# manyeyes/K2TransducerAsr

Hardware: AMD Instinct MI355X
Metric: RTFx (audio-sec/wall-sec) offline Zipformer greedy (higher is better)
Workload: dtype f32

## Files before the change

### k2transducerasr_amd/csrc/engine.cpp

```cpp
#include <cstring>
#include <thread>

#include "engine.h"
#include "lattice_ref.h"
#include "ctc_lattice_ref.h"
#include "ctc_prefix_bias_ref.h"
#include "ctc_prefix_ref.h"
#include "hotwords.h"
#include "ngram_lm.h"

#include <climits>
#include <cmath>

namespace k2hip {

namespace {
constexpr int kTailFrames = 19;
}

Engine::Engine(const std::string& weights, const char* overrides, int device) : device_(device) {
    tunables_init_from_env();
    model_.reset(new Model(weights, overrides));
    int n = 0;
    if (hipGetDeviceCount(&n) != hipSuccess || n <= 0)
// ... 208 lines not shown
        K2_HIP(hipMemcpyAsync(d_y, y.data(), sizeof(long long) * y.size(), hipMemcpyHostToDevice, stream_));
        Ctx t;
        t.stream = stream_;
        decoder_rows_wide(t, w, d_y, N, d_out);
        K2_HIP(hipMemcpyAsync(got.data(), d_out, sizeof(float) * got.size(), hipMemcpyDeviceToHost, stream_));
        K2_HIP(hipStreamSynchronize(stream_));
        for (int n = 0; n < N; n++) {
            const long long row = (y[2 * n] + 1) * V + y[2 * n + 1];
            K2_HIP(copy_blocking(want.data(), w.dec_table + row * w.J, sizeof(float) * w.J, hipMemcpyDeviceToHost));
            for (int k = 0; k < w.J; k++) *mismatched += memcmp(&want[k], &got[(size_t)n * w.J + k], sizeof(float)) != 0;
        }
    } catch (...) {
        (void)hipFree(d_y);
        (void)hipFree(d_out);
        throw;
    }
    (void)hipFree(d_y);
    (void)hipFree(d_out);
}

float* Engine::encoder_embed(const Ctx& c, const float* x, int B, int T, int* T50) {
    const Model& m = *model_;
    const int F0 = 80, T1 = T - 2, T2 = (T1 - 3) / 2 + 1, F2 = (F0 - 3) / 2 + 1, T3 = T2 - 2, F3 = (F2 - 3) / 2 + 1;
    K2_REQUIRE(T3 > 0, "encoder: %d input frames are too few (need >= 9)", T);
    Arena& ar = *c.arena;
    const int D0 = m.cfg().dim[0];
    float* out = ar.take<float>((int64_t)B * T3 * D0);
    int64_t mark = ar.mark();
    float* a1 = ar.take<float>((int64_t)B * T1 * F0 * 8);
    conv0_swoosh(c, x, m.w("encoder_embed.conv.0.weight"), m.w("encoder_embed.conv.0.bias"), a1, B, T, F0);
    c.add_flops(0, 2.0 * B * T1 * (double)F0 * 8 * 9, 0);
    float* a2 = ar.take<float>((int64_t)B * T2 * F2 * 32);
    {
        GemmArgs g;
        g.A = a1; g.W = m.w("encoder_embed.conv.4.weight#ohwi"); g.ldw = 72; g.bias = m.w("encoder_embed.conv.4.bias");
        g.C = a2; g.ldc = 32; g.M = B * T2 * F2; g.N = 32; g.K = 72; g.act = ACT_SWOOSH_R;
        g.cv_Fout = F2; g.cv_Tout = T2; g.cv_Tin = T1; g.cv_Fin = F0; g.cv_C = 8; g.cv_st = 2; g.cv_sf = 2;
        g.seg_len = 24; g.seg_stride = F0 * 8;
        gemm(c, g);
    }
    float* a3 = ar.take<float>((int64_t)B * T3 * F3 * 128);
    {
        GemmArgs g;
        g.A = a2; g.W = m.w("encoder_embed.conv.7.weight#ohwi"); g.ldw = 288; g.bias = m.w("encoder_embed.conv.7.bias");
        g.C = a3; g.ldc = 128; g.M = B * T3 * F3; g.N = 128; g.K = 288; g.act = ACT_SWOOSH_R;
        g.cv_Fout = F3; g.cv_Tout = T3; g.cv_Tin = T2; g.cv_Fin = F2; g.cv_C = 32; g.cv_st = 1; g.cv_sf = 2;
        g.seg_len = 96; g.seg_stride = F2 * 32;
        gemm(c, g);
    }
    const int npix = B * T3 * F3;
    float* dw = ar.take<float>((int64_t)npix * 128);
    dwconv7x7(c, a3, m.w("encoder_embed.convnext.depthwise_conv.weight#kc"), m.w("encoder_embed.convnext.depthwise_conv.bias"),
              dw, B, T3, T3, 3, F3, 128);
    float* hid = ar.take<float>((int64_t)npix * 384);
    linear(c, dw, 128, m.w("encoder_embed.convnext.pointwise_conv1.weight"), m.w("encoder_embed.convnext.pointwise_conv1.bias"),
           hid, 384, npix, 128, 384, ACT_SWOOSH_L);
    linear(c, hid, 384, m.w("encoder_embed.convnext.pointwise_conv2.weight"), m.w("encoder_embed.convnext.pointwise_conv2.bias"),
           a3, 128, npix, 384, 128, ACT_NONE, a3, 128);
    float* lin = ar.take<float>((int64_t)B * T3 * D0);
    linear(c, a3, F3 * 128, m.w("encoder_embed.out.weight#fc"), m.w("encoder_embed.out.bias"), lin, D0, B * T3, F3 * 128, D0);
    biasnorm(c, lin, m.w("encoder_embed.out_norm.bias"), m.w("encoder_embed.out_norm.log_scale"), out, B * T3, D0);
    ar.rewind(mark);
    *T50 = T3;
    return out;
}

const float* Engine::pos_proj_cached(const Ctx& c, int layer, const float* pe, int pe_dim, const float* W, int rows, int ncols) {
    if (c.dry) return nullptr;
    std::lock_guard<std::mutex> lk(cache_mu_);
    const auto key = std::make_pair(layer, rows);
    auto it = pp_cache_.find(key);
    if (it != pp_cache_.end()) return it->second;
    const size_t bytes = sizeof(float) * (size_t)rows * ncols;
    if (pp_cache_bytes_ + bytes > ((size_t)1 << 30)) {
        synchronize();
        for (auto& kv : pp_cache_) (void)hipFree(kv.second);
        pp_cache_.clear();
        pp_cache_bytes_ = 0;
    }
    float* pp = nullptr;
    K2_HIP(hipMalloc(&pp, bytes));
    Ctx plain = c;
    plain.instrument = false;
    plain.gemm_log = nullptr;
    linear(plain, pe, pe_dim, W, nullptr, pp, ncols, rows, pe_dim, ncols);
    K2_HIP(hipStreamSynchronize(c.stream));
    pp_cache_[key] = pp;
    pp_cache_bytes_ += bytes;
    return pp;
}

void Engine::encoder_layer(const Ctx& c, int si, int li, int gl, float* x, const float* pe, int B, int T, const StreamSite* site,
                           const LayerTail* tail) {
    const Model& m = *model_;
    const Config& cf = m.cfg();
    const int D = cf.dim[si], F = cf.ff[si], H = cf.heads[si], vh = cf.vhd[si], K = cf.kern[si], qh = cf.qhd[si], ph = cf.phd[si];
    const int L = site ? cf.left[si] : 0, M = B * T, KL = L + T, KLp = (KL + 3) & ~3, inproj = (2 * qh + ph) * H, Hc = 3 * D / 4, HV = H * vh;
    char p[96];
    snprintf(p, sizeof p, "encoder.encoders.%d.layers.%d.", si, li);
    auto w = [&](const char* suffix) { return m.w(std::string(p) + suffix); };
    auto wk = [&](const char* fmt, int k) {
        char name[96];
        snprintf(name, sizeof name, fmt, k);
        return w(name);
    };
    Arena& ar = *c.arena;
    int64_t mark = ar.mark();
    const long long SS = lay_.floats_per_stream;
    auto ring = [&](long long off) {
        RingRef r;
        r.pool = online_pool_; r.slot_stride = SS; r.off = off; r.slots = site->d_slots; r.chunks = site->d_chunks;
// ... 1583 lines not shown
            if (kcat) attn_stream(c, qkp, ld, kcat, pp, plen, aw, B, Tc, Lc, KLp, H, ds, left50);
            else attn_stream_ring(c, qkp, ld, r, pp, plen, aw, B, Tc, Lc, KLp, H, ds, left50);
        } else if (name == "glu_causal_conv") {
            float *x2 = P(), *pool = P();
            const long long ss = L(), off = L();
            const int* slots = reinterpret_cast<const int*>(P());
            float *wc = P(), *bc = P(), *ww = P(), *bw = P(), *sc = P(), *y = P();
            const int B = I(), Tc = I(), D = I(), K = I();
            glu_causal_conv(c, x2, pool, ss, off, slots, wc, bc, ww, bw, sc, y, B, Tc, D, K);
        } else if (name == "gemm") {
            GemmArgs g;
            g.M = I(); g.N = I(); g.K = I();
            g.lda = I(); g.ldw = I(); g.ldc = I(); g.ldr = I();
            g.act = I(); g.act_cols = I(); g.w_kn = I();
            g.nb0 = I(); g.nb1 = I();
            g.sA0 = L(); g.sA1 = L(); g.sW0 = L(); g.sW1 = L(); g.sC0 = L(); g.sC1 = L(); g.sR0 = L(); g.sR1 = L();
            g.sBias0 = L();
            g.cv_Fout = I(); g.cv_Tout = I(); g.cv_Tin = I(); g.cv_Fin = I(); g.cv_C = I(); g.cv_st = I(); g.cv_sf = I();
            g.seg_len = I(); g.seg_stride = I();
            g.res_div = I(); g.act_after_res = I();
            g.glu = I(); g.glu_cols = I();
            g.ldm = I(); g.sM0 = L(); g.sM1 = L();
            g.ld_orig = I();
            const int cfg = I(), res_is_C = I();
            const long long oA = L(), oW = L(), oR = L(), oC = L(), oM = L(), oO = L();
            float *A = P(), *W = P(), *bias = P(), *res = P(), *C = P();
            const int* skip = reinterpret_cast<const int*>(P());
            float *mul = P(), *orig = P(), *scale = P();
            int* plan_out = reinterpret_cast<int*>(P());
            K2_REQUIRE(A && W && C && plan_out && buf_bytes[n_bufs - 1] >= 20, "debug_op_run gemm: A, W, C and a plan buffer of 5 ints are needed");
            K2_REQUIRE(!(res_is_C && res), "debug_op_run gemm: res_is_C takes no res buffer");
            K2_REQUIRE(oA >= 0 && oW >= 0 && oR >= 0 && oC >= 0 && oM >= 0 && oO >= 0, "debug_op_run gemm: negative offset");
            if (res_is_C) res = C;
            g.A = A + oA; g.W = W + oW; g.bias = bias; g.res = res ? res + oR : nullptr; g.C = C + oC;
            g.skip_if_zero = skip;
            g.mul = mul ? mul + oM : nullptr;
            g.byp_orig = orig ? orig + oO : nullptr; g.byp_scale = scale;
            GemmForceGuard force(cfg);
            const GemmPlan pl = plan_gemm(g, gemm_force());
            const int rep[5] = {(int)pl.family, pl.idx, pl.BM, pl.BN, pl.mode};
            K2_HIP(copy_blocking(plan_out, rep, sizeof rep, hipMemcpyHostToDevice));
            gemm(c, g);
        } else if (name == "gemm_glu_causal_conv") {
            float *x = P(), *wg = P(), *bg = P(), *pool = P();
            const long long ss = L(), off = L();
            const int* slots = reinterpret_cast<const int*>(P());
            float *wc = P(), *bc = P(), *ww = P(), *bw = P(), *sc = P(), *y = P();
            const int B = I(), Tc = I(), D = I(), K = I();
            int* entry_out = reinterpret_cast<int*>(P());
            K2_REQUIRE(entry_out && buf_bytes[n_bufs - 1] >= 4, "debug_op_run gemm_glu_causal_conv: an entry buffer of 1 int is needed");
            const int entry = glu_conv_ring_entry(B, Tc, D, K);
            K2_HIP(copy_blocking(entry_out, &entry, sizeof entry, hipMemcpyHostToDevice));
            took = gemm_glu_causal_conv(c, x, wg, bg, pool, ss, off, slots, wc, bc, ww, bw, sc, y, B, Tc, D, K);
        } else if (name == "biasnorm") {
            float *x = P(), *bias = P(), *ls = P(), *y = P();
            const int M = I(), D = I();
            biasnorm(c, x, bias, ls, y, M, D);
        } else if (name == "bypass") {
            float *orig = P(), *x = P(), *scale = P(), *y = P();
            const int M = I(), D = I();
            bypass(c, orig, x, scale, y, M, D);
        } else if (name == "biasnorm_bypass") {
            float *x = P(), *orig = P(), *nb = P(), *ls = P(), *scale = P(), *y = P();
            const int M = I(), D = I();
            biasnorm_bypass(c, x, orig, nb, ls, scale, y, M, D);
        } else if (name == "biasnorm_bypass_downsample") {
            float *x = P(), *orig = P(), *nb = P(), *ls = P(), *scale = P(), *y = P(), *bias2 = P(), *xd2 = P();
            const int B = I(), T = I(), D = I(), ds2 = I(), D2 = I();
            biasnorm_bypass_downsample(c, x, orig, nb, ls, scale, y, bias2, xd2, B, T, D, ds2, D2);
        } else if (name == "downsample") {
            float *x = P(), *bias = P(), *y = P();
            const int B = I(), T = I(), D = I(), ds = I(), Din = I();
            downsample(c, x, bias, y, B, T, D, ds, Din);
        } else if (name == "downsample_full") {
            FullDimSegs s;
            s.n = I();
            K2_REQUIRE(s.n >= 1 && s.n <= 8, "debug_op_run downsample_full: %d segments", s.n);
            for (int k = 0; k < s.n; k++) s.ld[k] = I();
            for (int k = 0; k < s.n; k++) s.col1[k] = I();
            s.lz_Td = I(); s.lz_ds = I(); s.lz_Do = I();
            for (int k = 0; k < s.n; k++) s.src[k] = P();
            s.lz_orig = P(); s.lz_xd = P(); s.lz_scale = P();
            float *bias = P(), *y = P();
            const int B = I(), T = I(), D = I(), ds = I();
            downsample_full(c, s, bias, y, B, T, D, ds);
        } else if (name == "upsample_combine") {
            float *orig = P(), *xd = P(), *scale = P(), *y = P();
            const int B = I(), T = I(), Td = I(), D = I(), ds = I(), Dorig = I();
            upsample_combine(c, orig, xd, scale, y, B, T, Td, D, ds, Dorig);
        } else if (name == "upsample_combine_downsample") {
            float *orig = P(), *xd = P(), *scale = P(), *y = P(), *bias2 = P(), *xd2 = P();
            const int B = I(), T = I(), Td = I(), D = I(), ds = I(), Dorig = I(), D2 = I(), ds2 = I();
            upsample_combine_downsample(c, orig, xd, scale, y, bias2, xd2, B, T, Td, D, ds, Dorig, D2, ds2);
        } else if (name == "glu_dwconv1d_swoosh" || name == "glu_dwconv1d_dswish" || name == "dwconv1d_swoosh") {
            float *x = P(), *w = P(), *b = P(), *y = P();
            const int B = I(), T = I(), D = I(), K = I();
            if (name == "glu_dwconv1d_swoosh") glu_dwconv1d_swoosh(c, x, w, b, y, B, T, D, K);
            else if (name == "glu_dwconv1d_dswish") glu_dwconv1d_dswish(c, x, w, b, y, B, T, D, K);
            else dwconv1d_swoosh(c, x, w, b, y, B, T, D, K);
        } else if (name == "dwconv7x7") {
            float *x = P(), *w = P(), *b = P(), *y = P();
            const int B = I(), Tin = I(), Tout = I(), tpad = I(), F = I(), C = I();
            dwconv7x7(c, x, w, b, y, B, Tin, Tout, tpad, F, C);
        } else if (name == "conformer_qprep") {
            float *qkv = P(), *bu = P(), *bv = P(), *qu = P(), *qv = P();
            const int M = I(), D = I();
// ... 545 lines not shown
```

### k2transducerasr_amd/csrc/gemm.hip

```cpp
#include <algorithm>
#include <cmath>
#include <cstdlib>
#include <map>
#include <mutex>
#include <type_traits>

#include "act.h"
#include "kernels.h"

#pragma clang diagnostic ignored "-Winline-asm"

namespace k2hip {

typedef float f32x16 __attribute__((ext_vector_type(16)));
typedef float f32x4 __attribute__((ext_vector_type(4)));

namespace {


__device__ __forceinline__ float apply_act(float v, int act) {
    switch (act) {
        case ACT_SWOOSH_L: return swoosh_l(v);
        case ACT_SWOOSH_R: return swoosh_r(v);
        case ACT_TANH: {
// ... 1316 lines not shown
#undef K2_STAMP
}

template <int NT, int NW = 4>
__global__ __launch_bounds__(64 * NW) void gemm_f32_mfma_skinny(GemmArgs g) {
    if (g.skip_if_zero && *g.skip_if_zero == 0) return;
    __shared__ __attribute__((aligned(16))) float red[NW][NT][64][4];
    const int tid = threadIdx.x, lane = tid & 63, wave = tid >> 6;
    const int r = lane & 15, q = lane >> 4;
    const int m0 = blockIdx.x * 16, n0 = blockIdx.y * (16 * NT);
    const int Kw = g.K / NW, kbeg = wave * Kw;
    const float* __restrict__ ap = g.A + (long long)min(m0 + r, g.M - 1) * g.lda + kbeg + 4 * q;
    const float* __restrict__ wp[NT];
#pragma unroll
    for (int j = 0; j < NT; j++) wp[j] = g.W + (long long)min(n0 + 16 * j + r, g.N - 1) * g.ldw + kbeg + 4 * q;
    f32x4 acc[NT];
#pragma unroll
    for (int j = 0; j < NT; j++) acc[j] = f32x4{0.f, 0.f, 0.f, 0.f};
    constexpr int UN = NT <= 3 ? 4 : 2;
    for (int k = 0; k < Kw; k += 16 * UN) {
        float4 a4[UN], w4[UN][NT];
#pragma unroll
        for (int u = 0; u < UN; u++) {
            const int kk = min(k + 16 * u, Kw - 16);
            const float m = (k + 16 * u < Kw) ? 1.f : 0.f;
            a4[u] = *reinterpret_cast<const float4*>(ap + kk);
            a4[u].x *= m; a4[u].y *= m; a4[u].z *= m; a4[u].w *= m;
#pragma unroll
            for (int j = 0; j < NT; j++) w4[u][j] = *reinterpret_cast<const float4*>(wp[j] + kk);
        }
#pragma unroll
        for (int u = 0; u < UN; u++)
#pragma unroll
            for (int e = 0; e < 4; e++)
#pragma unroll
                for (int j = 0; j < NT; j++) {
                    const float av = e == 0 ? a4[u].x : e == 1 ? a4[u].y : e == 2 ? a4[u].z : a4[u].w;
                    const float bv = e == 0 ? w4[u][j].x : e == 1 ? w4[u][j].y : e == 2 ? w4[u][j].z : w4[u][j].w;
                    acc[j] = __builtin_amdgcn_mfma_f32_16x16x4f32(av, bv, acc[j], 0, 0, 0);
                }
    }
#pragma unroll
    for (int j = 0; j < NT; j++) *reinterpret_cast<f32x4*>(&red[wave][j][lane][0]) = acc[j];
    __syncthreads();
    for (int j = wave; j < NT; j += NW) {
        float vals[4];
#pragma unroll
        for (int e = 0; e < 4; e++) {
            float v = red[0][j][lane][e] + red[1][j][lane][e] + red[2][j][lane][e] + red[3][j][lane][e];
            if (NW == 8) v += (red[4][j][lane][e] + red[5][j][lane][e]) + (red[6][j][lane][e] + red[7][j][lane][e]);
            vals[e] = v;
        }
        epilogue_rows<4, Rows16>(g, vals, m0 + 4 * q, n0 + 16 * j + r, g.C, g.res, vals, false, nullptr, g.bias);
    }
}

template <int BM, int BN, int WM, int WN, int NST = 3>
void launch_dma(const Ctx& ctx, const GemmArgs& a) {
    dim3 grid(cdiv(a.N, BN), cdiv(a.M, BM), a.nb0 * a.nb1);
    size_t lds = sizeof(float) * NST * (BM + BN) * 32;
    static LdsAttrOnce lds_attr;
    lds_attr.ensure(gemm_f32_mfma_dma<BM, BN, WM, WN, NST>, (int)lds);
    hipLaunchKernelGGL((gemm_f32_mfma_dma<BM, BN, WM, WN, NST>), grid, dim3(64 * (BM / WM) * (BN / WN)), lds, ctx.stream, a);
}

template <int BM, int BN, int KS, int NST, int LW, int PF = 0>
void launch_ring(const Ctx& ctx, const GemmArgs& a) {
    dim3 grid(cdiv(a.N, BN), cdiv(a.M, BM), a.nb0 * a.nb1);
    size_t lds = sizeof(float) * std::max((size_t)NST * KS * (BM + BN) * 32, KS > 1 ? (size_t)KS * (BM / 32) * (BN / 32) * 1024 : (size_t)0) + (PF ? 256 : 0);
    static LdsAttrOnce lds_attr;
    lds_attr.ensure(gemm_f32_mfma_ring<BM, BN, KS, NST, LW, PF>, (int)lds);
    hipLaunchKernelGGL((gemm_f32_mfma_ring<BM, BN, KS, NST, LW, PF>), grid, dim3(64 * ((BM / 32) * (BN / 32) * KS + LW + PF)), lds, ctx.stream, a);
}

template <int BM, int BN, int KS, int NST, int PF = 0>
void launch_ring_conv(const Ctx& ctx, const GemmArgs& a) {
    dim3 grid(cdiv(a.N, BN), cdiv(a.M, BM), 1);
    const int pad = a.cf_K >> 1, Kc = (a.cf_K + 1) >> 1, CH = BN / 2;
    const size_t conv_fl = (size_t)(BM / a.cf_Tc) * CH * (pad + a.cf_Tc) + (size_t)CH * (Kc | 1) + (size_t)CH * a.cf_K;
    size_t lds = sizeof(float) * std::max({(size_t)NST * KS * (BM + BN) * 32, KS > 1 ? (size_t)KS * (BM / 32) * (BN / 32) * 1024 : (size_t)0, conv_fl}) + (PF ? 256 : 0);
    static LdsAttrOnce lds_attr;
    lds_attr.ensure(gemm_f32_mfma_ring<BM, BN, KS, NST, 0, PF, true>, (int)lds);
    hipLaunchKernelGGL((gemm_f32_mfma_ring<BM, BN, KS, NST, 0, PF, true>), grid, dim3(64 * ((BM / 32) * (BN / 32) * KS + PF)), lds, ctx.stream, a);
}

template <int BM, int BN, int WM, int WN, int NST>
void launch_pipe(const Ctx& ctx, const GemmArgs& a) {
    dim3 grid(cdiv(a.N, BN), cdiv(a.M, BM), 1);
    size_t lds = sizeof(float) * NST * (BM + BN) * 32;
    static LdsAttrOnce lds_attr;
    lds_attr.ensure(gemm_f32_mfma_pipe<BM, BN, WM, WN, NST>, (int)lds);
    K2_REQUIRE((long long)a.M * a.lda < (1ll << 29) && (long long)a.N * a.ldw < (1ll << 29), "pipe: operand too large for 31-bit lane byte offsets");
    K2_REQUIRE(a.K % 32 == 0 && a.K >= 32 * (NST - 1), "pipe: K %d too short for %d stages", a.K, NST);
    hipLaunchKernelGGL((gemm_f32_mfma_pipe<BM, BN, WM, WN, NST>), grid, dim3(64 * (BM / WM) * (BN / WN)), lds, ctx.stream, a);
}

template <int BM, int BN, int WM, int WN, int NST>
void launch_p16(const Ctx& ctx, const GemmArgs& a) {
    dim3 grid(cdiv(a.N, BN), cdiv(a.M, BM), 1);
    size_t lds = sizeof(float) * NST * (BM + BN) * 32;
    static LdsAttrOnce lds_attr;
    lds_attr.ensure(gemm_f32_mfma_p16<BM, BN, WM, WN, NST>, (int)lds);
    K2_REQUIRE((long long)a.M * a.lda < (1ll << 29) && (long long)a.N * a.ldw < (1ll << 29), "p16: operand too large for 31-bit lane byte offsets");
    K2_REQUIRE(a.K % 32 == 0 && a.K >= 32 * (NST - 1) && !a.glu, "p16: K %d too short for %d stages, or a gated epilogue", a.K, NST);
    hipLaunchKernelGGL((gemm_f32_mfma_p16<BM, BN, WM, WN, NST>), grid, dim3(64 * (BM / WM) * (BN / WN)), lds, ctx.stream, a);
}
// ... 81 lines not shown
            }
            break;
        case GemmFamily::SKINNY3:
            hipLaunchKernelGGL(gemm_f32_mfma_skinny<3>, dim3(cdiv(a.M, 16), 1), dim3(256), 0, ctx.stream, b);
            break;
        case GemmFamily::SKINNY6:
            hipLaunchKernelGGL(gemm_f32_mfma_skinny<6>, dim3(cdiv(a.M, 16), cdiv(a.N, 96)), dim3(256), 0, ctx.stream, b);
            break;
        case GemmFamily::SKINNY6_8:
            hipLaunchKernelGGL((gemm_f32_mfma_skinny<6, 8>), dim3(cdiv(a.M, 16), cdiv(a.N, 96)), dim3(512), 0, ctx.stream, b);
            break;
    }
    K2_HIP(hipGetLastError());
    if (ctx.instrument && ctx.gemm_log)
        ctx.gemm_log->push_back({a.M, a.N, a.K, a.nb0 * a.nb1, a.act, a.res != nullptr, gemm_kind(a, p), 0.f});
    if (ctx.instrument) K2_HIP(hipEventRecord(ctx.next_event(), ctx.stream));
}

bool gemm_glu_causal_conv(const Ctx& ctx, const float* x, const float* wg, const float* bg, float* pool, long long slot_stride, long long off,
                          const int* slots, const float* wc, const float* bc, const float* ww, const float* bw, const float* sc, float* y, int B,
                          int Tc, int D, int K) {
    const int M = B * Tc, N = 2 * D;
    const int entry = glu_conv_ring_entry(B, Tc, D, K);
    if (entry < 0) return false;
    const double fl = 2.0 * M * (double)N * D;
    ctx.add_flops(fl, 2.0 * M * (double)D * (K + (K + 1) / 2), 1);
    if (ctx.dry) return true;
    GemmArgs g;
    g.A = x; g.lda = D; g.W = wg; g.ldw = D; g.bias = bg; g.C = y; g.ldc = D; g.M = M; g.N = N; g.K = D;
    g.cf_pool = pool; g.cf_stride = slot_stride; g.cf_off = off; g.cf_slots = slots;
    g.cf_wc = wc; g.cf_bc = bc; g.cf_ww = ww; g.cf_bw = bw; g.cf_sc = sc; g.cf_Tc = Tc; g.cf_K = K;
    g.xcd_panels = tunables().xcd_panels;
    if (ctx.instrument) K2_HIP(hipEventRecord(ctx.next_event(), ctx.stream));
    if (ctx.instrument && ctx.gemm_log) ctx.gemm_log->push_back({M, N, D, 1, 0, 0, 64, 0.f});
    switch (entry) {
        case 16: launch_ring_conv_entry<16>(ctx, g); break;
        case 17: launch_ring_conv_entry<17>(ctx, g); break;
        case 12: launch_ring_conv_entry<12>(ctx, g); break;
        default: launch_ring_conv_entry<8>(ctx, g); break;
    }
    K2_HIP(hipGetLastError());
    if (ctx.instrument) K2_HIP(hipEventRecord(ctx.next_event(), ctx.stream));
    return true;
}

void linear(const Ctx& ctx, const float* A, int lda, const float* W, const float* bias, float* C, int ldc, int M, int K,
            int N, int act, const float* res, int ldr) {
    GemmArgs g;
    g.A = A; g.lda = lda; g.W = W; g.ldw = K; g.bias = bias; g.C = C; g.ldc = ldc;
    g.M = M; g.N = N; g.K = K; g.act = act; g.res = res; g.ldr = ldr;
    gemm(ctx, g);
}

}
```

### k2transducerasr_amd/csrc/kernels.h

```cpp
#pragma once
#include "ctc_prefix_layout.h"
#include "common.h"

namespace k2hip {

#ifdef K2HIP_DEV
#define K2HIP_DEV_SWITCH(name, def) int name = def
#else
#define K2HIP_DEV_SWITCH(name, def) static constexpr int name = def
#endif
struct Tunables {
    int no_glu_epilogue = 0;
    int attn_long = 0;
    int no_fused_av = 0;
    int fused_vproj_min_t = 4;
    int no_fused_vproj = 0;
    int no_fused_conv = 0;
    int conformer_gemm_scores = 0;
    int dw7_tiled = 0;
    int dw1d_tt = 0;
    int lstm_seq = 0;
    int greedy_one_part = 0;
    int greedy_parts = 0;
    int beam_launches = 0;
    int beam_parts = 0;
    int beam_hyp_global = 0;
    int beam_trace = 0;
    int search_rounds = -1;
    int test_greedy_timeout = 0;
    int decoder_table_mb = 1024;
    int screen_min_v = 1024;
    int screen_count = 0;
    int max_streams = 0;
    K2HIP_DEV_SWITCH(gemm_cfg, -1);
    K2HIP_DEV_SWITCH(xcd_panels, 0);
    K2HIP_DEV_SWITCH(greedy_stamps, 0);
    K2HIP_DEV_SWITCH(conformer_stamps, 0);
};
void tunables_init_from_env();
const Tunables& tunables();
bool tunables_set(const char* env_name, int value);

struct GemmStats {
    double flops = 0;
    double total_flops = 0;
    int launches = 0;
    float ms = 0;
};

struct GemmLaunchRec {
    int M, N, K, batch, act, res, kind;
    float us;
};

struct GreedyLaunch;
struct Ctx {
    std::vector<GemmLaunchRec>* gemm_log = nullptr;
    GreedyLaunch* greedy_rec = nullptr;
    hipStream_t stream = nullptr;
    Arena* arena = nullptr;
    bool dry = false;
    bool one_part = false;
    bool instrument = false;
    GemmStats* stats = nullptr;
    std::vector<hipEvent_t>* evpool = nullptr;
    int* evused = nullptr;
    hipEvent_t next_event() const {
        if ((size_t)*evused == evpool->size()) {
            hipEvent_t e;
            K2_HIP(hipEventCreate(&e));
// ... 56 lines not shown
#define K2_PIPE_TABLE(X)                                                                                                       \
    X(0, 128, 64, 64, 32, 3) X(1, 128, 64, 32, 32, 3) X(2, 128, 128, 64, 64, 3) X(3, 128, 128, 64, 32, 3) X(4, 128, 64, 64, 32, 4)  \
    X(5, 64, 64, 32, 32, 3) X(6, 128, 128, 64, 64, 4) X(7, 64, 128, 32, 64, 3) X(8, 128, 128, 32, 32, 3) X(9, 128, 64, 32, 32, 4) \
    X(10, 64, 64, 64, 32, 3) X(11, 64, 64, 32, 64, 3) X(12, 256, 64, 64, 32, 3) X(13, 128, 32, 32, 32, 3) X(14, 128, 32, 64, 32, 3)
#define K2_P16_TABLE(X) X(0, 64, 96, 32, 48, 3) X(1, 128, 96, 64, 48, 3) X(2, 64, 192, 32, 96, 3) X(3, 32, 96, 16, 48, 3)
#define K2_RING_TABLE(X)                                                                                        \
    X(0, 128, 64, 1, 2, 0, 0) X(1, 128, 64, 1, 3, 0, 0) X(2, 128, 64, 1, 2, 0, 1) X(3, 128, 64, 1, 3, 0, 1) X(4, 128, 64, 1, 4, 0, 1)   \
    X(5, 64, 64, 1, 3, 0, 0) X(6, 64, 64, 1, 3, 0, 1) X(7, 64, 64, 1, 4, 0, 1) X(8, 64, 64, 2, 3, 0, 0) X(9, 64, 64, 2, 3, 0, 1)      \
    X(10, 64, 64, 4, 2, 0, 0) X(11, 64, 64, 4, 2, 0, 1) X(12, 32, 64, 2, 3, 0, 0) X(13, 32, 64, 4, 3, 0, 0) X(14, 32, 64, 4, 3, 0, 1)  \
    X(15, 32, 32, 4, 3, 0, 0) X(16, 32, 32, 4, 4, 0, 1) X(17, 64, 32, 4, 3, 0, 0) X(18, 128, 128, 1, 2, 0, 0) X(19, 128, 128, 1, 2, 0, 1) \
    X(20, 64, 128, 1, 3, 0, 0) X(21, 64, 128, 1, 3, 0, 1) X(22, 64, 96, 1, 3, 0, 0) X(23, 64, 96, 1, 3, 0, 1) X(24, 128, 96, 1, 2, 0, 1) \
    X(25, 128, 64, 1, 3, 2, 0) X(26, 128, 64, 1, 3, 2, 1) X(27, 128, 64, 2, 2, 0, 1) X(28, 64, 96, 2, 3, 0, 0) X(29, 64, 96, 2, 2, 0, 0) \
    X(30, 64, 96, 2, 2, 0, 1) X(31, 128, 96, 1, 3, 0, 0) X(32, 128, 96, 1, 3, 0, 1)
struct RingCfg { int BM, BN, KS, NST, LW, PF; };
#define X(i, bm, bn, ks, nst, lw, pf) {bm, bn, ks, nst, lw, pf},
constexpr RingCfg kRing[] = {K2_RING_TABLE(X)};
#undef X
#define K2_DMA_TABLE(X)                                                                                                          \
    X(0, 128, 128, 64, 32, 3) X(5, 128, 64, 32, 32, 2) X(8, 128, 64, 32, 32, 4) X(9, 64, 64, 32, 32, 2) X(10, 64, 64, 32, 32, 3) \
    X(11, 64, 96, 32, 32, 2) X(20, 32, 32, 32, 32, 4) X(21, 32, 64, 32, 32, 4)
#define K2_REG_TABLE(X)                                                                                                           \
    X(0, 128, 128, 64, 32, 32) X(1, 128, 128, 64, 32, 64) X(2, 64, 64, 32, 32, 32) X(3, 64, 64, 32, 32, 64) X(4, 128, 64, 32, 32, 64) \
    X(5, 128, 64, 32, 32, 32) X(12, 128, 32, 32, 32, 32)
enum GemmMode { MODE_PLAIN = 0, MODE_CONV = 1, MODE_WKN = 2 };

enum class GemmFamily { REG, DMA, PIPE, P16, RING, SKINNY3, SKINNY6, SKINNY6_8 };
struct GemmPlan {
    GemmFamily family = GemmFamily::REG;
    int idx = 0;
    int mode = MODE_PLAIN;
    int ablate = 0;
    int BM = 0, BN = 0, waves = 0;
};
struct GemmForce {
    enum Kind { AUTO, CFG, RING, PIPE, P16 } kind = AUTO;
    int idx = -1;
    int ablate = 0;
    bool dma = true;
};
GemmForce decode_gemm_force(int code);
GemmPlan plan_gemm(const GemmArgs& a, const GemmForce& f);
int gemm_kind(const GemmArgs& a, const GemmPlan& p);
int glu_conv_ring_entry(int B, int Tc, int D, int K);
void debug_force_gemm_cfg(int code);
GemmForce gemm_force();
struct GemmForceGuard {
    explicit GemmForceGuard(int code) { debug_force_gemm_cfg(code); }
    ~GemmForceGuard() { debug_force_gemm_cfg(-1); }
    GemmForceGuard(const GemmForceGuard&) = delete;
    GemmForceGuard& operator=(const GemmForceGuard&) = delete;
};
void linear(const Ctx& ctx, const float* A, int lda, const float* W, const float* bias, float* C, int ldc, int M, int K,
            int N, int act = ACT_NONE, const float* res = nullptr, int ldr = 0);

struct RingRef {
    float* pool = nullptr;
    long long slot_stride = 0;
    long long off = 0;
    const int* slots = nullptr;
    const int* chunks = nullptr;
};

void attn_scores_softmax(const Ctx& ctx, const float* qkp, int ld, const float* pp, float* aw, int B, int T, int Tp, int H, int qh = 32,
                         int koff0 = -1, int poff0 = -1);

bool attn_av_out(const Ctx& ctx, const float* aw, const float* v, const float* wout, const float* bias, float* x, int B, int T, int KL, int Tp,
                 int H, int vh, int D);
bool attn_av_out_ring(const Ctx& ctx, const float* aw, const RingRef& vals, const float* newrows, const float* wout, const float* bias, float* x,
                      int B, int T, int KL, int Tp, int H, int vh, int D);
void attn_proj_av_out_ring(const Ctx& ctx, const float* aw, const RingRef& vals, const float* xin, const float* win, const float* bin,
                           const float* wout, const float* bias, float* xout, int B, int T, int KL, int Tp, int H, int vh, int D);

void nonlin_av_out_ring(const Ctx& ctx, const float* aw, const RingRef& cache, const float* hid, int ldh, const float* wout, const float* bias,
                        float* x, int B, int T, int KL, int Tp, int Hc, int D);

void pad_logfloor(const Ctx& ctx, const float* packed, const long long* d_off, const long long* d_len, float* out, int B,
                  long long L);
void pad_logfloor_dense(const Ctx& ctx, const float* feats, long long n_each, float* out, int B, long long L);
void conv0_swoosh(const Ctx& ctx, const float* x, const float* w, const float* b, float* y, int B, int T, int F);
void act_forms(const Ctx& ctx, const float* x, float* y_lean, float* y_libm, int act, long long n);
void conv0_pad1_dswish(const Ctx& ctx, const float* x, const float* w, const float* b, float* y, int B, int T, int F);
void dwconv7x7(const Ctx& ctx, const float* x, const float* w_kc, const float* b, float* y, int B, int Tin, int Tout, int tpad,
               int F, int C);
void biasnorm(const Ctx& ctx, const float* x, const float* bias, const float* log_scale, float* y, int M, int D);
void biasnorm_bypass(const Ctx& ctx, const float* x, const float* orig, const float* nbias, const float* log_scale,
                     const float* scale, float* y, int M, int D);
void biasnorm_bypass_downsample(const Ctx& ctx, const float* x, const float* orig, const float* nbias, const float* log_scale, const float* scale,
                                float* y, const float* bias2, float* xd2, int B, int T, int D, int ds2, int D2);
struct LayerTail {
    const float* bias2 = nullptr;
    float* xd2 = nullptr;
    int ds2 = 1, D2 = 0;
};
void bypass(const Ctx& ctx, const float* orig, const float* x, const float* scale, float* y, int M, int D);
void glu_sigmoid(const Ctx& ctx, const float* x, float* y, int M, int D);
void tanh_gate(const Ctx& ctx, const float* x, float* y, int M, int Hc);
void dwconv1d_swoosh(const Ctx& ctx, const float* x, const float* w_kd, const float* b, float* y, int B, int T, int D, int K);
void glu_dwconv1d_swoosh(const Ctx& ctx, const float* x2, const float* w_kd, const float* b, float* y, int B, int T, int D,
                          int K);
void glu_dwconv1d_dswish(const Ctx& ctx, const float* x2, const float* w_kd, const float* b, float* y, int B, int T, int D,
                          int K);
void conv0_nopad_dswish(const Ctx& ctx, const float* x, const float* w, const float* b, float* y, int B, int T, int F);
void lstm_cell(const Ctx& ctx, const float* gx, long long ldgx, const float* gh, int ldgh, float* c, float* hf, int B, int Hh);
void add_inplace(const Ctx& ctx, float* a, const float* b, long long n);
void lstm_cell_rows(const Ctx& ctx, const float* gates, float* c, float* hf, int rows, int Hh);
void lstm_add_frame(const Ctx& ctx, const float* Y, long long SY, const float* hp, long long pstride, int S, float* h, float* x1, int n, int B,
// ... 343 lines not shown
```

### k2transducerasr_amd/csrc/online_engine.cpp

```cpp
#include <climits>
#include <cmath>

#include "engine.h"
#include "ctc_prefix_ref.h"

namespace k2hip {

void Engine::online_ensure_pool() {
    if (online_pool_) return;
    const Config& c = model_->cfg();
    K2_REQUIRE(c.streaming || c.lstm, "this model is not a streaming export (metadata 'streaming' != 1)");
    OnlineLayout& L = lay_;
    long long off = 0;
    if (c.conformer) {
        L.nl = c.nlayer[0];
        L.floats_per_stream = ((long long)c.nlayer[0] * (c.left[0] + c.kern[0] - 1) * c.dim[0] + 63) / 64 * 64;
        online_cap_ = 256;
        if (tunables().max_streams > 0) online_cap_ = tunables().max_streams;
        K2_HIP(hipSetDevice(device_));
        K2_HIP(hipMalloc(&online_pool_, sizeof(float) * (size_t)L.floats_per_stream * online_cap_));
        for (int i = online_cap_ - 1; i >= 0; i--) free_slots_.push_back(i);
        return;
    }
    if (c.lstm) {
// ... 161 lines not shown
    const float cl = sqrtf((float)pd), ls = (float)pd / (2.0f * (float)M_PI), logcl = logf(cl);
    for (int n = 0; n < n2; n++) {
        float x = (float)(n - (Tc + L - 1));
        float sg = (float)((x > 0.f) - (x < 0.f));
        float xa = atanf(cl * sg * (logf(fabsf(x) + cl) - logcl) / ls);
        for (int k = 0; k < pd / 2; k++) {
            pe[(size_t)n * pd + 2 * k] = cosf(xa * (float)(k + 1));
            pe[(size_t)n * pd + 2 * k + 1] = sinf(xa * (float)(k + 1));
        }
        pe[(size_t)n * pd + pd - 1] = 1.0f;
    }
    float* d = nullptr;
    K2_HIP(hipMalloc(&d, pe.size() * sizeof(float)));
    K2_HIP(copy_blocking(d, pe.data(), pe.size() * sizeof(float), hipMemcpyHostToDevice));
    pe_cache_[key] = d;
    return d;
}

float* Engine::encoder_embed_stream(const Ctx& c, const float* x, const int* d_slots, int B, int T, int* Tc_out) {
    const Model& m = *model_;
    const int F0 = 80, T1 = T - 2, T2 = (T1 - 3) / 2 + 1, F2 = (F0 - 3) / 2 + 1, T3 = T2 - 2, F3 = (F2 - 3) / 2 + 1, Tc = T3 - 3;
    K2_REQUIRE(Tc > 0 && F3 == 19, "streaming embed: chunk of %d frames unsupported", T);
    Arena& ar = *c.arena;
    const int D0 = m.cfg().dim[0];
    float* out = ar.take<float>((int64_t)B * Tc * D0);
    int64_t mark = ar.mark();
    float* a1 = ar.take<float>((int64_t)B * T1 * F0 * 8);
    conv0_swoosh(c, x, m.w("encoder_embed.conv.0.weight"), m.w("encoder_embed.conv.0.bias"), a1, B, T, F0);
    float* a2 = ar.take<float>((int64_t)B * T2 * F2 * 32);
    {
        GemmArgs g;
        g.A = a1; g.W = m.w("encoder_embed.conv.4.weight#ohwi"); g.ldw = 72; g.bias = m.w("encoder_embed.conv.4.bias");
        g.C = a2; g.ldc = 32; g.M = B * T2 * F2; g.N = 32; g.K = 72; g.act = ACT_SWOOSH_R;
        g.cv_Fout = F2; g.cv_Tout = T2; g.cv_Tin = T1; g.cv_Fin = F0; g.cv_C = 8; g.cv_st = 2; g.cv_sf = 2;
        g.seg_len = 24; g.seg_stride = F0 * 8;
        gemm(c, g);
    }
    float* a3 = ar.take<float>((int64_t)B * T3 * F3 * 128);
    {
        GemmArgs g;
        g.A = a2; g.W = m.w("encoder_embed.conv.7.weight#ohwi"); g.ldw = 288; g.bias = m.w("encoder_embed.conv.7.bias");
        g.C = a3; g.ldc = 128; g.M = B * T3 * F3; g.N = 128; g.K = 288; g.act = ACT_SWOOSH_R;
        g.cv_Fout = F3; g.cv_Tout = T3; g.cv_Tin = T2; g.cv_Fin = F2; g.cv_C = 32; g.cv_st = 1; g.cv_sf = 2;
        g.seg_len = 96; g.seg_stride = F2 * 32;
        gemm(c, g);
    }
    float* cat = ar.take<float>((int64_t)B * (T3 + 3) * F3 * 128);
    const int npix = B * Tc * F3;
    float* byp = ar.take<float>((int64_t)npix * 128);
    convnext_cat(c, a3, online_pool_, lay_.floats_per_stream, lay_.embed, d_slots, cat, byp, B, T3, Tc, F3, 128);
    float* dw = ar.take<float>((int64_t)npix * 128);
    dwconv7x7(c, cat, m.w("encoder_embed.convnext.depthwise_conv.weight#kc"), m.w("encoder_embed.convnext.depthwise_conv.bias"), dw, B,
              T3 + 3, Tc, 0, F3, 128);
    float* hid = ar.take<float>((int64_t)npix * 384);
    linear(c, dw, 128, m.w("encoder_embed.convnext.pointwise_conv1.weight"), m.w("encoder_embed.convnext.pointwise_conv1.bias"), hid, 384,
           npix, 128, 384, ACT_SWOOSH_L);
    linear(c, hid, 384, m.w("encoder_embed.convnext.pointwise_conv2.weight"), m.w("encoder_embed.convnext.pointwise_conv2.bias"), byp, 128,
           npix, 384, 128, ACT_NONE, byp, 128);
    float* lin = ar.take<float>((int64_t)B * Tc * D0);
    linear(c, byp, F3 * 128, m.w("encoder_embed.out.weight#fc"), m.w("encoder_embed.out.bias"), lin, D0, B * Tc, F3 * 128, D0);
    biasnorm(c, lin, m.w("encoder_embed.out_norm.bias"), m.w("encoder_embed.out_norm.log_scale"), out, B * Tc, D0);
    ar.rewind(mark);
    *Tc_out = Tc;
    return out;
}

float* Engine::online_encoder_zip2(const Ctx& c, const float* d_x, const int* d_slots, const long long* d_plen, const int* d_chunks, int B) {
    const int Tp = online_frames_per_chunk();
    int Tc = 0;
    float* x = encoder_embed_stream(c, d_x, d_slots, B, model_->cfg().chunk_T, &Tc);
    K2_REQUIRE((Tc + 1) / 2 == Tp, "internal: chunk yields %d frames, expected %d", (Tc + 1) / 2, Tp);
    const StreamSite site{d_slots, d_plen, d_chunks};
    FullDimSegs segs;
    encoder_stacks(c, x, B, Tc, &site, -1, nullptr, nullptr, &segs);
    return encoder_head(c, segs, B, Tc, nullptr);
}

void Engine::online_step(const int* slots, const float* const* chunks, const long long* hyps, const long long* plens, const int* nchunks, int B,
                         int64_t* tokens, int32_t* ts, int32_t* n_tokens, const int* fifo_heads) {
    online_step_impl(slots, chunks, hyps, plens, nchunks, B, tokens, ts, n_tokens, fifo_heads, nullptr);
}
void Engine::online_step_beam(const int* slots, const float* const* chunks, const long long* plens, const int* nchunks, int B, int K,
                              const int* beam_in, int* beam_out, const int* fifo_heads) {
    K2_REQUIRE(K >= 1 && K <= kMaxBeam, "online beam search: beam %d out of range [1,%d]", K, kMaxBeam);
    K2_REQUIRE(!model_->cfg().ctc, "online beam search: a CTC model runs its own search");
    std::vector<long long> hyps(2 * (size_t)B, K2HIP_BLANK_ID);
    OnlineBeamIO io{K, beam_in, beam_out, nullptr};
    online_step_impl(slots, chunks, hyps.data(), plens, nchunks, B, nullptr, nullptr, nullptr, fifo_heads, &io);
}
void Engine::online_step_beam_hw(const int* slots, const float* const* chunks, const long long* plens, const int* nchunks, int B, int K,
                                 const int* beam_in, int* beam_out, const BeamHwIO& hw, const int* fifo_heads) {
    K2_REQUIRE(K >= 1 && K <= kMaxBeam, "online beam search: beam %d out of range [1,%d]", K, kMaxBeam);
    K2_REQUIRE(!model_->cfg().ctc, "online beam search: a CTC model runs its own search");
    std::vector<long long> hyps(2 * (size_t)B, K2HIP_BLANK_ID);
    OnlineBeamIO io{K, beam_in, beam_out, &hw};
    online_step_impl(slots, chunks, hyps.data(), plens, nchunks, B, nullptr, nullptr, nullptr, fifo_heads, &io);
}
void Engine::online_step_ctc_prefix(const int* slots, const float* const* chunks, const long long* plens, const int* nchunks, int B, int K,
                                    const int* cp_in, int* cp_out, const int* fifo_heads) {
    K2_REQUIRE(K >= 1 && K <= kMaxBeam, "online ctc prefix search: beam %d out of range [1,%d]", K, kMaxBeam);
    K2_REQUIRE(model_->cfg().ctc, "online ctc prefix search: the model has no CTC head");
    const CtcPrefixResumeLayout L{K, online_frames_per_chunk()};
    ctc_prefix_chunk_check_args(B, L.Tc, model_->cfg().V, nullptr, K, cp_in, L.in_ints(), L.in_e(), L.in_rel());
    std::vector<long long> hyps(2 * (size_t)B, K2HIP_BLANK_ID);
    OnlineCtcPrefixIO io{K, cp_in, cp_out};
    online_step_impl(slots, chunks, hyps.data(), plens, nchunks, B, nullptr, nullptr, nullptr, fifo_heads, nullptr, &io);
}
void Engine::online_step_impl(const int* slots, const float* const* chunks, const long long* hyps, const long long* plens, const int* nchunks,
                              int B, int64_t* tokens, int32_t* ts, int32_t* n_tokens, const int* fifo_heads, const OnlineBeamIO* beam,
                              const OnlineCtcPrefixIO* cpx) {
    online_ensure_pool();
// ... 146 lines not shown
```

### k2transducerasr_amd/csrc/tunables.cpp

```cpp
#include <cstdlib>
#include <cstring>
#include <mutex>

#include "kernels.h"

namespace k2hip {

namespace {
constexpr int kMaxDev = 64;
std::mutex g_util_mu[kMaxDev];
hipStream_t g_util_stream[kMaxDev] = {};
hipError_t util_device(int* dev) {
    hipError_t e = hipGetDevice(dev);
    if (e != hipSuccess) return e;
    return (*dev < 0 || *dev >= kMaxDev) ? hipErrorInvalidDevice : hipSuccess;
}
hipError_t util_stream(int dev, hipStream_t* s) {
    if (!g_util_stream[dev]) {
        hipError_t e = hipStreamCreateWithFlags(&g_util_stream[dev], hipStreamNonBlocking);
        if (e != hipSuccess) return e;
    }
    *s = g_util_stream[dev];
    return hipSuccess;
}
}
hipError_t copy_blocking(void* dst, const void* src, size_t bytes, hipMemcpyKind kind) {
    if (bytes == 0) return hipSuccess;
    int dev = 0;
    hipError_t e = util_device(&dev);
    if (e != hipSuccess) return e;
    std::lock_guard<std::mutex> lk(g_util_mu[dev]);
    hipStream_t s = nullptr;
    e = util_stream(dev, &s);
    if (e != hipSuccess) return e;
    e = hipMemcpyAsync(dst, src, bytes, kind, s);
    if (e != hipSuccess) return e;
    return hipStreamSynchronize(s);
}
hipError_t fill_blocking(void* dst, int value, size_t bytes) {
    if (bytes == 0) return hipSuccess;
    int dev = 0;
    hipError_t e = util_device(&dev);
    if (e != hipSuccess) return e;
    std::lock_guard<std::mutex> lk(g_util_mu[dev]);
    hipStream_t s = nullptr;
    e = util_stream(dev, &s);
    if (e != hipSuccess) return e;
    e = hipMemsetAsync(dst, value, bytes, s);
    if (e != hipSuccess) return e;
    return hipStreamSynchronize(s);
}

namespace {
Tunables g_t;
bool g_init = false;
struct Entry {
    const char* env;
    int Tunables::*field;
    bool flag;
};
const Entry kEntries[] = {
    {"K2HIP_NO_GLU_EPILOGUE", &Tunables::no_glu_epilogue, true},
    {"K2HIP_ATTN_LONG", &Tunables::attn_long, true},
    {"K2HIP_NO_FUSED_AV", &Tunables::no_fused_av, true},
    {"K2HIP_NO_FUSED_VPROJ", &Tunables::no_fused_vproj, true},
    {"K2HIP_FUSED_VPROJ_MIN_T", &Tunables::fused_vproj_min_t, false},
    {"K2HIP_NO_FUSED_CONV", &Tunables::no_fused_conv, true},
    {"K2HIP_CONFORMER_GEMM_SCORES", &Tunables::conformer_gemm_scores, true},
    {"K2HIP_DW7_TILED", &Tunables::dw7_tiled, true},
    {"K2HIP_DW1D_TT", &Tunables::dw1d_tt, false},
    {"K2HIP_LSTM_SEQ", &Tunables::lstm_seq, true},
    {"K2HIP_GREEDY_ONE_PART", &Tunables::greedy_one_part, true},
    {"K2HIP_GREEDY_PARTS", &Tunables::greedy_parts, false},
    {"K2HIP_DECODER_TABLE_MB", &Tunables::decoder_table_mb, false},
    {"K2HIP_BEAM_LAUNCHES", &Tunables::beam_launches, true},
    {"K2HIP_BEAM_HYP_GLOBAL", &Tunables::beam_hyp_global, true},
    {"K2HIP_BEAM_PARTS", &Tunables::beam_parts, false},
    {"K2HIP_BEAM_TRACE", &Tunables::beam_trace, true},
    {"K2HIP_SCREEN_MIN_V", &Tunables::screen_min_v, false},
    {"K2HIP_SCREEN_COUNT", &Tunables::screen_count, false},
    {"K2HIP_TEST_GREEDY_TIMEOUT", &Tunables::test_greedy_timeout, true},
    {"K2HIP_SEARCH_ROUNDS", &Tunables::search_rounds, false},
    {"K2HIP_MAX_STREAMS", &Tunables::max_streams, false},
#ifdef K2HIP_DEV
    {"K2HIP_GEMM_CFG", &Tunables::gemm_cfg, false},
    {"K2HIP_XCD_PANELS", &Tunables::xcd_panels, false},
    {"K2HIP_GREEDY_STAMPS", &Tunables::greedy_stamps, true},
    {"K2HIP_CONFORMER_STAMPS", &Tunables::conformer_stamps, true},
#endif
};
}

void tunables_init_from_env() {
    static std::once_flag once;
    std::call_once(once, [] {
    g_init = true;
    for (const Entry& e : kEntries)
        if (const char* v = getenv(e.env)) g_t.*(e.field) = e.flag ? 1 : atoi(v);
    });
}

const Tunables& tunables() { return g_t; }
bool tunables_set(const char* env_name, int value) {
    for (const Entry& e : kEntries)
        if (!strcmp(e.env, env_name)) {
            g_t.*(e.field) = value;
            return true;
        }
    return false;
}

}
```

Baseline: 23910.

## Fuse ConvNeXt pointwise conv pair into one MFMA kernel keeping hidden in registers

Adds a dedicated kernel that computes both ConvNeXt pointwise convolutions (128->384 SwooshL ->128 plus residual) in one pass. The 384-wide hidden activation stays in registers instead of round-tripping through global memory. Weight chunks are streamed into LDS with double-buffered direct-to-LDS loads. It is used when there are at least 32768 pixels, falling back to two GEMMs otherwise, and it adds hand-scheduled assembly with alignment requirements.

```diff
diff --git a/k2transducerasr_amd/csrc/engine.cpp b/k2transducerasr_amd/csrc/engine.cpp
--- a/k2transducerasr_amd/csrc/engine.cpp
+++ b/k2transducerasr_amd/csrc/engine.cpp
@@ -284,11 +284,8 @@
     float* dw = ar.take<float>((int64_t)npix * 128);
     dwconv7x7(c, a3, m.w("encoder_embed.convnext.depthwise_conv.weight#kc"), m.w("encoder_embed.convnext.depthwise_conv.bias"),
               dw, B, T3, T3, 3, F3, 128);
-    float* hid = ar.take<float>((int64_t)npix * 384);
-    linear(c, dw, 128, m.w("encoder_embed.convnext.pointwise_conv1.weight"), m.w("encoder_embed.convnext.pointwise_conv1.bias"),
-           hid, 384, npix, 128, 384, ACT_SWOOSH_L);
-    linear(c, hid, 384, m.w("encoder_embed.convnext.pointwise_conv2.weight"), m.w("encoder_embed.convnext.pointwise_conv2.bias"),
-           a3, 128, npix, 384, 128, ACT_NONE, a3, 128);
+    convnext_pointwise(c, dw, m.w("encoder_embed.convnext.pointwise_conv1.weight"), m.w("encoder_embed.convnext.pointwise_conv1.bias"),
+                       m.w("encoder_embed.convnext.pointwise_conv2.weight"), m.w("encoder_embed.convnext.pointwise_conv2.bias"), a3, npix, 128, 384);
     float* lin = ar.take<float>((int64_t)B * T3 * D0);
     linear(c, a3, F3 * 128, m.w("encoder_embed.out.weight#fc"), m.w("encoder_embed.out.bias"), lin, D0, B * T3, F3 * 128, D0);
     biasnorm(c, lin, m.w("encoder_embed.out_norm.bias"), m.w("encoder_embed.out_norm.log_scale"), out, B * T3, D0);
@@ -1978,6 +1975,11 @@
             const int entry = glu_conv_ring_entry(B, Tc, D, K);
             K2_HIP(copy_blocking(entry_out, &entry, sizeof entry, hipMemcpyHostToDevice));
             took = gemm_glu_causal_conv(c, x, wg, bg, pool, ss, off, slots, wc, bc, ww, bw, sc, y, B, Tc, D, K);
+        } else if (name == "convnext_pw_pair") {
+            float *x = P(), *w1 = P(), *b1 = P(), *w2 = P(), *b2 = P(), *io = P();
+            const long long npix = L();
+            K2_REQUIRE(x && w1 && b1 && w2 && b2 && io, "debug_op_run convnext_pw_pair: x, w1, b1, w2, b2 and io are needed");
+            took = convnext_pointwise_pair(c, x, w1, b1, w2, b2, io, npix, 128, 384);
         } else if (name == "biasnorm") {
             float *x = P(), *bias = P(), *ls = P(), *y = P();
             const int M = I(), D = I();
diff --git a/k2transducerasr_amd/csrc/gemm.hip b/k2transducerasr_amd/csrc/gemm.hip
--- a/k2transducerasr_amd/csrc/gemm.hip
+++ b/k2transducerasr_amd/csrc/gemm.hip
@@ -1392,6 +1392,143 @@
             vals[e] = v;
         }
         epilogue_rows<4, Rows16>(g, vals, m0 + 4 * q, n0 + 16 * j + r, g.C, g.res, vals, false, nullptr, g.bias);
+    }
+}
+
+constexpr int CNX_C = 128, CNX_H = 384, CNX_WAVES = 4, CNX_PIX = 32 * CNX_WAVES;
+constexpr int CNX_STAGE = 2 * 128 * 32;
+constexpr int CNX_IPW = (CNX_STAGE / 256) / CNX_WAVES;
+constexpr int CNX_LDS_BYTES = (2 * CNX_STAGE + CNX_H) * 4;
+static_assert(CNX_IPW * CNX_WAVES * 256 == CNX_STAGE && (CNX_IPW / 2) * CNX_WAVES == 16, "convnext pair: a wave's first half of DMAs is W1's image");
+
+__global__ __launch_bounds__(64 * CNX_WAVES, 2) void convnext_pw_pair_kernel(const float* __restrict__ x, const float* __restrict__ w1,
+                                                                              const float* __restrict__ b1, const float* __restrict__ w2,
+                                                                              const float* __restrict__ b2, float* io, int npix) {
+    extern __shared__ __attribute__((aligned(16))) float smem[];
+    const int tid = threadIdx.x;
+    const int lane = tid & 63, wave = __builtin_amdgcn_readfirstlane(tid >> 6);
+    const int li = lane & 31, lh = lane >> 5;
+    const long long px = (long long)blockIdx.x * CNX_PIX + wave * 32 + li;
+    const long long row = px < npix ? px : (long long)npix - 1;
+
+    const float* xp = x + row * CNX_C + 4 * lh;
+    f32x4 xf[16];
+#pragma unroll
+    for (int q = 0; q < 16; q++) xf[q] = *reinterpret_cast<const f32x4*>(xp + 8 * q);
+    if (tid < CNX_H / 4) *reinterpret_cast<f32x4*>(smem + 2 * CNX_STAGE + 4 * tid) = *reinterpret_cast<const f32x4*>(b1 + 4 * tid);
+
+    const unsigned lds_base = (unsigned)(unsigned long long)(__attribute__((address_space(3))) char*)smem;
+    unsigned voff[CNX_IPW];
+    unsigned long long sb[CNX_IPW];
+    unsigned mq[CNX_IPW];
+#pragma unroll
+    for (int q = 0; q < CNX_IPW; q++) {
+        const int inst = wave + q * CNX_WAVES;
+        const int slot = (inst & 15) * 64 + lane;
+        const int r = slot >> 3, cp = slot & 7;
+        const int ch = cp ^ ((r >> 1) & 7);
+        const bool is1 = q < CNX_IPW / 2;
+        voff[q] = (unsigned)((is1 ? (r & 31) * CNX_C + 32 * (r >> 5) + 4 * ch : r * CNX_H + 4 * ch) * 4);
+        const unsigned long long base = (unsigned long long)(is1 ? w1 : w2);
+        sb[q] = ((unsigned long long)(unsigned)__builtin_amdgcn_readfirstlane((int)(base >> 32)) << 32) |
+                (unsigned long long)(unsigned)__builtin_amdgcn_readfirstlane((int)(unsigned)base);
+        mq[q] = __builtin_amdgcn_readfirstlane(lds_base + inst * 1024);
+    }
+#define K2_CNX_DMA(ST_, C_, W1ON_, W2ON_)                                                                                  \
+    _Pragma("unroll") for (int q = 0; q < CNX_IPW; q++) {                                                                  \
+        if (q < CNX_IPW / 2 ? (W1ON_) : (W2ON_)) {                                                                         \
+            const unsigned long long src_ =                                                                                \
+                sb[q] + (q < CNX_IPW / 2 ? (unsigned long long)((C_) + 1) * (32 * CNX_C * 4) : (unsigned long long)(C_) * (32 * 4)); \
+            asm volatile("s_add_u32 m0, %2, %3\n\ts_nop 0\n\tglobal_load_lds_dwordx4 %0, %1"                                \
+                         :                                                                                                 \
+                         : "v"(voff[q]), "s"(src_), "s"(mq[q]), "n"((ST_) * CNX_STAGE * 4)                                  \
+                         : "memory", "m0", "scc");                                                                         \
+        }                                                                                                                  \
+    }
+    K2_CNX_DMA(1, -1, true, false)
+    K2_CNX_DMA(0, 0, true, true)
+
+    const int sw = (li >> 1) & 7;
+    const float* fr[4];
+#pragma unroll
+    for (int g = 0; g < 4; g++) fr[g] = smem + li * 32 + (((2 * g + lh) ^ sw) << 2);
+    const float* bl = smem + 2 * CNX_STAGE + 4 * lh;
+
+    f32x16 out[4];
+#pragma unroll
+    for (int i = 0; i < 4; i++)
+#pragma unroll
+        for (int r = 0; r < 16; r++) out[i][r] = 0.f;
+    f32x16 h, hn;
+
+#define K2_CNX_STEP1(ST_, H_)                                                                                              \
+    {                                                                                                                      \
+        _Pragma("unroll") for (int r = 0; r < 16; r++) H_[r] = 0.f;                                                        \
+        _Pragma("unroll") for (int kt = 0; kt < 4; kt++) _Pragma("unroll") for (int g = 0; g < 4; g++) {                   \
+            const f32x4 a = *reinterpret_cast<const f32x4*>(fr[g] + (ST_) * CNX_STAGE + kt * 1024);                        \
+            _Pragma("unroll") for (int e = 0; e < 4; e++) H_ = __builtin_amdgcn_mfma_f32_32x32x2f32(a[e], xf[4 * kt + g][e], H_, 0, 0, 0); \
+        }                                                                                                                  \
+    }
+#define K2_CNX_ITER(ST_, C_, NEXT_, DMA1_, DMA2_, PRE_)                                                                          \
+    {                                                                                                                      \
+        __builtin_amdgcn_sched_barrier(0);                                                                                 \
+        asm volatile("s_waitcnt vmcnt(0) lgkmcnt(0)" ::: "memory");                                                        \
+        __builtin_amdgcn_s_barrier();                                                                                      \
+        PRE_                                                                                                               \
+        __builtin_amdgcn_sched_barrier(0);                                                                                 \
+        if (NEXT_) K2_CNX_STEP1(ST_, hn)                                                                                   \
+        _Pragma("unroll") for (int g = 0; g < 4; g++) {                                                                    \
+            const f32x4 bv = *reinterpret_cast<const f32x4*>(bl + (C_) * 32 + 8 * g);                                      \
+            _Pragma("unroll") for (int e = 0; e < 4; e++) h[4 * g + e] = apply_act(h[4 * g + e] + bv[e], ACT_SWOOSH_L);    \
+        }                                                                                                                  \
+        if (NEXT_) {                                                                                                       \
+            _Pragma("unroll") for (int n = 0; n < 64; n++) {                                                               \
+                __builtin_amdgcn_sched_group_barrier(0x008, 1, 0);                                                         \
+                if (n < 20) __builtin_amdgcn_sched_group_barrier(0x100, 1, 0);                                             \
+                __builtin_amdgcn_sched_group_barrier(0x002, 4, 0);                                                         \
+            }                                                                                                              \
+        }                                                                                                                  \
+        __builtin_amdgcn_sched_barrier(0);                                                                                 \
+        _Pragma("unroll") for (int g = 0; g < 4; g++) {                                                                    \
+            f32x4 a[4];                                                                                                    \
+            _Pragma("unroll") for (int i = 0; i < 4; i++)                                                                  \
+                a[i] = *reinterpret_cast<const f32x4*>(fr[g] + (ST_) * CNX_STAGE + 4096 + i * 1024);                       \
+            _Pragma("unroll") for (int e = 0; e < 4; e++) _Pragma("unroll") for (int i = 0; i < 4; i++)                    \
+                out[i] = __builtin_amdgcn_mfma_f32_32x32x2f32(a[i][e], h[4 * g + e], out[i], 0, 0, 0);                     \
+            if (g == 0 && ((DMA1_) || (DMA2_))) {     \
+                __builtin_amdgcn_sched_barrier(0);                                                                         \
+                K2_CNX_DMA((ST_) ^ 1, (C_) + 1, DMA1_, DMA2_)                                                              \
+                __builtin_amdgcn_sched_barrier(0);                                                                         \
+            }                                                                                                              \
+        }                                                                                                                  \
+        if (NEXT_) h = hn;                                                                                                 \
+    }
+    float* iop = io + row * CNX_C + 4 * lh;
+    f32x4 rv[16];
+#define K2_CNX_RES _Pragma("unroll") for (int q = 0; q < 16; q++) rv[q] = *reinterpret_cast<const f32x4*>(iop + 8 * q);
+    asm volatile("s_waitcnt vmcnt(0) lgkmcnt(0)" ::: "memory");
+    __builtin_amdgcn_s_barrier();
+    K2_CNX_STEP1(1, h)
+    constexpr int NC = CNX_H / 32;
+    for (int c = 0; c < NC - 2; c += 2) {
+        K2_CNX_ITER(0, c, true, true, true, {})
+        K2_CNX_ITER(1, c + 1, true, true, true, {})
+    }
+    K2_CNX_ITER(0, NC - 2, true, false, true, {})
+    K2_CNX_ITER(1, NC - 1, false, false, false, K2_CNX_RES)
+#undef K2_CNX_ITER
+#undef K2_CNX_RES
+#undef K2_CNX_STEP1
+#undef K2_CNX_DMA
+
+    const float* b2p = b2 + 4 * lh;
+#pragma unroll
+    for (int q = 0; q < 16; q++) {
+        const f32x4 bv = *reinterpret_cast<const f32x4*>(b2p + 8 * q);
+        f32x4 v;
+#pragma unroll
+        for (int e = 0; e < 4; e++) v[e] = (out[q >> 2][4 * (q & 3) + e] + bv[e]) + rv[q][e];
+        if (px < npix) *reinterpret_cast<f32x4*>(iop + 8 * q) = v;
     }
 }
 
@@ -1579,4 +1716,29 @@
     gemm(ctx, g);
 }
 
-}
+bool convnext_pointwise_pair(const Ctx& ctx, const float* x, const float* w1, const float* b1, const float* w2, const float* b2, float* io,
+                             long long npix, int C, int hidden) {
+    if (C != CNX_C || hidden != CNX_H || npix < 1 || npix >= (1ll << 31) - CNX_PIX) return false;
+    if (!ctx.dry && ((((uintptr_t)x | (uintptr_t)w1 | (uintptr_t)b1 | (uintptr_t)w2 | (uintptr_t)b2 | (uintptr_t)io) & 15) != 0 || x == io)) return false;
+    ctx.add_flops(2.0 * npix * (double)CNX_H * CNX_C * 2, 0.0, 1);
+    if (ctx.dry) return true;
+    static LdsAttrOnce lds_attr;
+    lds_attr.ensure(convnext_pw_pair_kernel, CNX_LDS_BYTES);
+    if (ctx.instrument) K2_HIP(hipEventRecord(ctx.next_event(), ctx.stream));
+    if (ctx.instrument && ctx.gemm_log) ctx.gemm_log->push_back({(int)npix, CNX_C, 2 * CNX_H, 1, ACT_SWOOSH_L, 1, 8, 0.f});
+    hipLaunchKernelGGL(convnext_pw_pair_kernel, dim3(cdiv(npix, CNX_PIX)), dim3(64 * CNX_WAVES), CNX_LDS_BYTES, ctx.stream, x, w1, b1, w2, b2, io,
+                       (int)npix);
+    K2_HIP(hipGetLastError());
+    if (ctx.instrument) K2_HIP(hipEventRecord(ctx.next_event(), ctx.stream));
+    return true;
+}
+
+void convnext_pointwise(const Ctx& ctx, const float* x, const float* w1, const float* b1, const float* w2, const float* b2, float* io,
+                        long long npix, int C, int hidden) {
+    if (npix >= 32768 && !tunables().no_fused_convnext && convnext_pointwise_pair(ctx, x, w1, b1, w2, b2, io, npix, C, hidden)) return;
+    float* hid = ctx.arena->take<float>(npix * hidden);
+    linear(ctx, x, C, w1, b1, hid, hidden, (int)npix, C, hidden, ACT_SWOOSH_L);
+    linear(ctx, hid, hidden, w2, b2, io, C, (int)npix, hidden, C, ACT_NONE, io, C);
+}
+
+}
diff --git a/k2transducerasr_amd/csrc/kernels.h b/k2transducerasr_amd/csrc/kernels.h
--- a/k2transducerasr_amd/csrc/kernels.h
+++ b/k2transducerasr_amd/csrc/kernels.h
@@ -16,6 +16,7 @@
     int fused_vproj_min_t = 4;
     int no_fused_vproj = 0;
     int no_fused_conv = 0;
+    int no_fused_convnext = 0;
     int conformer_gemm_scores = 0;
     int dw7_tiled = 0;
     int dw1d_tt = 0;
@@ -178,6 +179,10 @@
 };
 void linear(const Ctx& ctx, const float* A, int lda, const float* W, const float* bias, float* C, int ldc, int M, int K,
             int N, int act = ACT_NONE, const float* res = nullptr, int ldr = 0);
+bool convnext_pointwise_pair(const Ctx& ctx, const float* x, const float* w1, const float* b1, const float* w2, const float* b2, float* io,
+                             long long npix, int C, int hidden);
+void convnext_pointwise(const Ctx& ctx, const float* x, const float* w1, const float* b1, const float* w2, const float* b2, float* io,
+                        long long npix, int C, int hidden);
 
 struct RingRef {
     float* pool = nullptr;
diff --git a/k2transducerasr_amd/csrc/online_engine.cpp b/k2transducerasr_amd/csrc/online_engine.cpp
--- a/k2transducerasr_amd/csrc/online_engine.cpp
+++ b/k2transducerasr_amd/csrc/online_engine.cpp
@@ -237,11 +237,8 @@
     float* dw = ar.take<float>((int64_t)npix * 128);
     dwconv7x7(c, cat, m.w("encoder_embed.convnext.depthwise_conv.weight#kc"), m.w("encoder_embed.convnext.depthwise_conv.bias"), dw, B,
               T3 + 3, Tc, 0, F3, 128);
-    float* hid = ar.take<float>((int64_t)npix * 384);
-    linear(c, dw, 128, m.w("encoder_embed.convnext.pointwise_conv1.weight"), m.w("encoder_embed.convnext.pointwise_conv1.bias"), hid, 384,
-           npix, 128, 384, ACT_SWOOSH_L);
-    linear(c, hid, 384, m.w("encoder_embed.convnext.pointwise_conv2.weight"), m.w("encoder_embed.convnext.pointwise_conv2.bias"), byp, 128,
-           npix, 384, 128, ACT_NONE, byp, 128);
+    convnext_pointwise(c, dw, m.w("encoder_embed.convnext.pointwise_conv1.weight"), m.w("encoder_embed.convnext.pointwise_conv1.bias"),
+                       m.w("encoder_embed.convnext.pointwise_conv2.weight"), m.w("encoder_embed.convnext.pointwise_conv2.bias"), byp, npix, 128, 384);
     float* lin = ar.take<float>((int64_t)B * Tc * D0);
     linear(c, byp, F3 * 128, m.w("encoder_embed.out.weight#fc"), m.w("encoder_embed.out.bias"), lin, D0, B * Tc, F3 * 128, D0);
     biasnorm(c, lin, m.w("encoder_embed.out_norm.bias"), m.w("encoder_embed.out_norm.log_scale"), out, B * Tc, D0);
diff --git a/k2transducerasr_amd/csrc/tunables.cpp b/k2transducerasr_amd/csrc/tunables.cpp
--- a/k2transducerasr_amd/csrc/tunables.cpp
+++ b/k2transducerasr_amd/csrc/tunables.cpp
@@ -66,6 +66,7 @@
     {"K2HIP_NO_FUSED_VPROJ", &Tunables::no_fused_vproj, true},
     {"K2HIP_FUSED_VPROJ_MIN_T", &Tunables::fused_vproj_min_t, false},
     {"K2HIP_NO_FUSED_CONV", &Tunables::no_fused_conv, true},
+    {"K2HIP_NO_FUSED_CONVNEXT", &Tunables::no_fused_convnext, true},
     {"K2HIP_CONFORMER_GEMM_SCORES", &Tunables::conformer_gemm_scores, true},
     {"K2HIP_DW7_TILED", &Tunables::dw7_tiled, true},
     {"K2HIP_DW1D_TT", &Tunables::dw1d_tt, false},
```

After: 24080 (median of 6 runs). No clear change (+0.7%).
